# waiwera/waiwera

Measured on AMD Instinct MI355X. Metric: Newton steps/sec, 10M-cell eos_we (BCSR SpMV GB/s in roofline), higher is better.
Workload: dtype f64

## Files before the change

### waiwera_amd/csrc/context.hpp

```cpp
#pragma once
#include <hip/hip_runtime.h>
#include <string>
#include <type_traits>
#include <vector>
#include "../../include/waiwera_hip.h"
#include "devbuf.hpp"
#include "ilu_schedule.hpp"
#include "mesh_pattern.hpp"
#include "physics.hip.h"
#include "tile_schedule.hpp"

namespace wai {

__host__ __device__ __forceinline__ size_t ell_ld(size_t n) {
  size_t ld = (n + 511) & ~(size_t)511;
  if ((ld & 262143) == 0) ld += 512;
  return ld;
}
__host__ __device__ __forceinline__ size_t ell_rows(int bs, size_t n) {
  if (bs >= 3) return ell_ld(n);
  return n;
}
__host__ __device__ __forceinline__ size_t ell_ix1(int bs, size_t n, int r, int k, size_t i) {
  if (bs >= 3) return ((i >> 6) * (size_t)(bs * bs) + (size_t)(r * bs + k)) * 64 + (i & 63);
// ... 226 lines not shown
constexpr int MAX_TRACERS = 8;
constexpr int POST_OFF = 64;
constexpr unsigned long long POST_KEY = 0x5bd1e995a5a5c3c3ull;
struct Tracers {
  int nt = 0;
  int phase[MAX_TRACERS] = {0};
  double decay[MAX_TRACERS] = {0}, activation[MAX_TRACERS] = {0}, diffusion[MAX_TRACERS] = {0};
  double* bc = nullptr;
  double* inj = nullptr;
  double* rhsb = nullptr;
  int mode = 0;
  long long n_sweeps = 0;
  unsigned char kernarg_tail[136] = {0};
};
static_assert(sizeof(Tracers) == 408, "Tracers is a kernel argument (k_tracer_assemble_all, k_tracer_lhs): its size is part of their argument layout");
static_assert(std::is_trivially_copyable<Tracers>::value, "a kernel argument holds views, never an owner");

struct TracerForm {
  int method, it, nt, phase;
  double dt, ratio, decay, activation, diffusion;
};
static_assert(std::is_trivially_copyable<TracerForm>::value && std::is_trivially_copyable<ResForm>::value &&
              std::is_trivially_copyable<EosParams>::value, "a kernel argument holds views, never an owner");

constexpr int FIN_MAXF = 64;
struct Fin {
  int count = 0;
  int nb = 0;
  int nf = 1;
  double* part2 = nullptr;
  int slot0 = 0, nslots = 0;
  int phase = -1;
  int seq = 0;
  double* scal = nullptr;
  double* post = nullptr;
};
static_assert(std::is_trivially_copyable<Fin>::value, "a kernel argument holds views, never an owner");

struct Krylov {
  double* d_post = nullptr;
  int seq = 0;
  long long n_launch = 0, n_copy = 0;
  DevBuf<double> partials;
  DevBuf<double> partials2;
  DevBuf<unsigned> started;
  bool alpha_pending = false;
  int nb_max = 0;
  DevBuf<double> scal;
  PinnedBuf<double> h_scal;
  int nblocks = 0;
  int nb_pc = 0;
};

struct KrylovVecs {
  DevBuf<double> R, RP, P, V, S, T, tmp, X_own;
  double* X = nullptr;
  DevBuf<double> bl;
  DevBuf<double> basis;
  int basis_m = 0;
};

struct KspOpts {
  int type = WAI_KSP_BCGS, restart = 30, max_its = 10000;
  double rtol = 1.e-5, atol = 1.e-50;
};
struct PcOpts {
  int type = WAI_AUX_PC_FOLLOW, asm_overlap = 1, ilu_levels = 0, sub = WAI_SUB_ILU;
};

struct LinSys {
  Bcsr A;
  DevBuf<double> val, fdg;
  KspOpts ksp;
  PcOpts pc;
  int n = 0, nl = 0;
  KrylovVecs* kv = nullptr;
  AsmSystem as;
  bool net_blocks = false;
};

struct Gather {
  DevBuf<double> in;
  DevBuf<double> send;
  DevBuf<double> recv;
  DevBuf<double> out;
  DevBuf<double> counts;
  DevBuf<int> idx;
  DevBuf<int> claim;
  DevBuf<int> flag;
  size_t n_in = 0, n_send = 0, n_recv = 0, n_out = 0, n_counts = 0, n_idx = 0, n_claim = 0;
};

}

namespace wai {
struct LuBlocks {
  DevBuf<double> inv;
  DevBuf<size_t> inv_ptr;
  std::vector<size_t> h_inv_ptr;
  size_t total = 0;
  int bs = 0;
};
int launch_lu_apply(wai_ctx* c, int bs, const double* r, double* z);

struct Handles {
  hipStream_t stream = nullptr;
  Comm* comm = nullptr;
  hipEvent_t ev_scal = nullptr;
  hipStream_t comm_stream = nullptr;
  hipEvent_t ev_pack = nullptr, ev_halo = nullptr;
  hipEvent_t ev0 = nullptr, ev1 = nullptr, pev0 = nullptr, pev1 = nullptr;
  Handles() = default;
  Handles(const Handles&) = delete;
  ~Handles();
};
}

struct wai_ctx : wai::Handles {
  int device = 0;
  int n_cu = 256;
  size_t lds_per_block = 64 * 1024;
  int kind = 0, np = 0, df = 0, nmob = 0;
  bool salt = false;
  wai::EosParams ep{};
  wai_solver_opts opts{};
  int sub_pc = WAI_SUB_ILU;
  std::vector<int> pc_tiles;
  wai::DeviceMesh mesh;
  wai::Sources src;
  wai::Network net;
  std::vector<int> src_gidx;
  int src_nglobal = 0;
  wai::Pattern pat;
  wai::LinSys flow, aux, coupled;
  wai::KrylovVecs kv, kv_coupled;
  wai::IluSchedule ilu;
  wai::LuBlocks lu;
  wai::Krylov ks;
  wai::Tracers tr;
  wai::Gather gat;
  wai::DevBuf<double> tr_bc, tr_inj, tr_rhsb;
  wai::DevBuf<double> flu, flu_last_iter, flu_last_step, flu_pert;
  wai::DevBuf<double> hstep;
  wai::DevBuf<double> w_y, w_yold, w_delta, w_f, w_lhs, w_a, w_b, w_c;
  wai::DevBuf<int> d_flags;
  wai::PinnedBuf<int> h_flags;
  wai::DevBuf<double> d_red;
  wai::PinnedBuf<double> h_red;
  wai::DevBuf<double> stage[4];
  size_t stage_len = 0;
  struct EnvSw {
    bool fin_separate = false; bool no_col16 = false; bool scalar_kernels = false; bool iluk_level_path = false;
    bool asm_unfused = false; bool no_desc_share = false; bool no_pack = false;
  } env;
  int test_drop_wait = 0;
  int n_nbr = 0;
  std::vector<int> nbr_rank, send_ptr, recv_ptr;
  wai::DevBuf<int> d_send_idx; wai::DevBuf<double> d_sendbuf, d_recvbuf;
  int send_total = 0, max_dof_buf = 0;
  double fnorm0 = 0.0;
  int method = 0;
  double ratio = 0.0;
  wai::DevBuf<double> w_lhs2;
  int scheme = 0, taken = 0;
  double dt_last = 0.0;
  wai::DevBuf<double> w_hist;
  wai::DevBuf<double> w_hist_prev;
  double dt_last_prev = 0.0;
  bool can_reject = false;
  bool prof_on = false;
  bool last_iter_partial = false;
  double prof_ms[wai::KC_COUNT] = {0};
  long long prof_n[wai::KC_COUNT] = {0};
  std::string err;
  bool bc_set = false;
  int dbg = 0;
};

namespace wai {
int launch_eos(wai_ctx* c, const double* y, int first, int count, bool perturbed);
int launch_residual(wai_ctx* c, double dt, const double* lhs_old, double* f, double* lhs_out,
                    double* rhs_out, const int* only = nullptr, int n_only = 0);
int launch_jacobian(wai_ctx* c, double dt, const double* lhs_old);
int launch_transitions(wai_ctx* c, const double* y_old, double* search, double* y);
int launch_tracer_assemble(wai_ctx* c, const TracerForm& tf, const double* alx_last,
                           const double* alx_last2, double* b);
int launch_tracer_assemble_all(wai_ctx* c, int method, double dt, double ratio, const double* alx_last,
                               const double* alx_last2, double* b);
int launch_tracer_lhs(wai_ctx* c, double* Al);
int launch_separator(wai_ctx* c, double pressure, double* out);
int launch_face_fluxes(wai_ctx* c, const int* face_cells, double* out);
int launch_source_rates(wai_ctx* c, double* out, bool raw = false);
int launch_tracer_pick(wai_ctx* c, const double* X, int it, double* x);
int launch_tracer_put(wai_ctx* c, const double* x, int it, double* X);
int launch_tracer_alx(wai_ctx* c, const double* X, double* alx);
int launch_max_scaled(wai_ctx* c, const double* v, const double* scale, double tol, double* val,
                      int* idx);
int launch_fluid_aos(wai_ctx* c, const double* flu_soa, double* out_aos);
int launch_region_get(wai_ctx* c, double* out);
int launch_region_set(wai_ctx* c, const double* in, int first, int count);

int launch_spmv(wai_ctx* c, const Bcsr& M, const double* x, double* y);
int launch_ilu_factor_on(wai_ctx* c, const Bcsr& M, IluSchedule& s);
int launch_pc_on(wai_ctx* c, const Bcsr& M, const IluSchedule& s, bool spmv, const double* in, double* z,
                 int dot_mode, const double* aux, const int* list = nullptr, int nrun = 0, const Fin* fin = nullptr,
                 const double* in2 = nullptr, const Bcsr* F = nullptr, const int* row_map = nullptr);
int pc_kernel_kind(const wai_ctx* c, const Bcsr& M, const IluSchedule& s);
bool pc_axpy_capable(const wai_ctx* c, const Bcsr& M);
bool pc_axpy_default(const wai_ctx* c, const Bcsr& M);
int launch_big_solve(wai_ctx* c, const Bcsr& M, const IluSchedule& s, double* z);
int launch_sublu_solve(wai_ctx* c, const Bcsr& M, const IluSchedule& s, double* z);
bool sublu_vector_in_lds(const IluSchedule& s, int bs);
int launch_asm_gather_matrix(wai_ctx* c, const Bcsr& M, const AsmSystem& a);
int launch_pack_rows(wai_ctx* c, const Bcsr& M);
int launch_unpack_rows(wai_ctx* c, const Bcsr& M, const AsmSystem& a);
int launch_asm_gather(wai_ctx* c, const AsmSystem& a, const double* r);
int launch_asm_scatter(wai_ctx* c, const AsmSystem& a, double* z);
int vec_dots(wai_ctx* c, const double* a1, const double* b1, int slot1, const double* a2, const double* b2,
             int slot2, int n);
int launch_pc(wai_ctx* c, const Bcsr& M, bool spmv, const double* in, double* z, int dot_mode, const double* aux,
              const int* list = nullptr, int nrun = 0, const Fin* fin = nullptr, const double* in2 = nullptr);
Fin make_fin(wai_ctx* c, int slot0, int nslots, int phase, bool post = false);
inline Fin make_fin_dots(wai_ctx* c, int dot_mode, int phase, bool post = false) {
  return make_fin(c, pc_dot_slot0(dot_mode), pc_dot_nslots(dot_mode), phase, post);
}
int launch_ell_to_bcsr(wai_ctx* c, const Bcsr& M, double* bcsr);
int launch_dg_spmv(wai_ctx* c, const Bcsr& M, const double* x, double* y);
int launch_dg_factor(wai_ctx* c, const Bcsr& M, IluSchedule& s);
int launch_dg_pc(wai_ctx* c, const Bcsr& M, const IluSchedule& s, bool spmv, const double* in, double* z, const int* list, int nrun);
int launch_dg_big_solve(wai_ctx* c, const Bcsr& M, const IluSchedule& s, double* z);
int launch_dg_to_bcsr(wai_ctx* c, const Bcsr& M, double* bcsr);
int launch_bcsr_to_ell(wai_ctx* c, const double* bcsr, const Bcsr& M);
int vec_finalize(wai_ctx* c, int nb, int slot0, int nslots, int phase);
int vec_dot(wai_ctx* c, const double* a, const double* b, int n, int slot);
int partials_clear(wai_ctx* c, int slot0, int nslots);
int vec_copy(wai_ctx* c, double* dst, const double* src, size_t n);
int vec_zero(wai_ctx* c, double* dst, size_t n);
int vec_waxpy(wai_ctx* c, double* w, double alpha, const double* x, const double* y, int n);
int bcgs_scalars(wai_ctx* c, int phase, bool post = false);
int bcgs_update_xrp_derive(wai_ctx* c, const KrylovVecs& k, int n);
int bcgs_post(wai_ctx* c, int seq);
void read_env(wai_ctx* c);
int test_drop_partials(wai_ctx* c, int n);
int bcgs_update_p(wai_ctx* c, const KrylovVecs& k, int n);
int bcgs_update_s(wai_ctx* c, const KrylovVecs& k, int n);
int bcgs_update_xr(wai_ctx* c, const KrylovVecs& k, int n, bool dots = true, int fin_phase = -2, bool post = false);
int bcgs_update_xrp(wai_ctx* c, const KrylovVecs& k, int n);
int pack_halo_axpy(wai_ctx* c, const double* a, const double* b, int dof, hipStream_t stream = nullptr);
int gmres_mdot(wai_ctx* c, const double* basis, size_t ld, int n, const double* w, int k);
int gmres_maxpy_norm(wai_ctx* c, const double* basis, size_t ld, int n, double* w, int k);
int gmres_scale_to(wai_ctx* c, double* dst, const double* src, int slot_norm2, int n);
int gmres_update_x(wai_ctx* c, const double* basis, size_t ld, int n, double* x, const double* ycoef_host, int k);
int pack_halo(wai_ctx* c, const double* vec, int dof, hipStream_t stream = nullptr);
int unpack_halo(wai_ctx* c, double* vec, int dof, hipStream_t stream = nullptr);
}
```

### waiwera_amd/csrc/kernels_fused.hip

```cpp
#include "pc_generic.hip.h"
#include "pc_wide.hip.h"
#include "pc_park.hip.h"
#include "pc_rows.hip.h"
#include "pc_wave.hip.h"
#include "krylov_vec.hip.h"

namespace wai {

static inline int vgrid(int n) {
  int g = (n + TPB - 1) / TPB;
  return g > 1024 ? 1024 : (g < 1 ? 1 : g);
}

void read_env(wai_ctx* c) {
  c->env.fin_separate = getenv("WAI_FIN_SEPARATE") != nullptr;
  c->env.no_col16 = getenv("WAI_NO_COL16") != nullptr;
  c->env.scalar_kernels = getenv("WAI_BCGS_SCALAR_KERNELS") != nullptr;
  c->env.iluk_level_path = getenv("WAI_ILUK_LEVEL_PATH") != nullptr;
  c->env.asm_unfused = getenv("WAI_ASM_UNFUSED") != nullptr;
  c->env.no_desc_share = getenv("WAI_NO_DESC_SHARE") != nullptr;
  c->env.no_pack = getenv("WAI_NO_PACK") != nullptr;
}

int pc_kernel_kind(const wai_ctx* c, const Bcsr& J, const IluSchedule& s) {
  if (J.dg) return -1;
  if (s.wide) return 4;
  if (c->dbg) return 0;
  if (s.wave_kernel && J.bs >= 3) return 3;
  if (s.rows_kernel) return 2;
  if (park_serves(s, J.bs)) return 1;
  return 0;
}
static bool kind_composes(int kind) { return kind >= 1 && kind <= 3; }
bool pc_axpy_capable(const wai_ctx* c, const Bcsr& M) { return !c->ilu.big && kind_composes(pc_kernel_kind(c, M, c->ilu)); }
bool pc_axpy_default(const wai_ctx* c, const Bcsr& M) {
  if (c->ilu.big) return false;
  const int kind = pc_kernel_kind(c, M, c->ilu);
  return (kind == 1 && c->ilu.col16 && !c->env.no_col16) || kind == 3;
}

template <int BS>
static void launch_pc_bs(wai_ctx* c, const Bcsr& J, const IluSchedule& s, bool spmv, const double* in, double* z,
                         int dot_mode, const double* aux, const int* list, int nrun, const Fin* finp, const double* in2,
                         const Bcsr* F, const int* row_map) {
  const int which = !list ? 0 : (list == s.sub_int ? 1 : (list == s.sub_bnd ? 2 : -1));
  if (!list) { nrun = s.nsub; list = s.sub_order; }
  const bool with_fin = finp && dot_mode != 0;
  Fin fin;
  if (finp && dot_mode != 0) { fin = *finp; fin.count = nrun; fin.nb = s.nsub; fin.nf = fin_slices(s.nsub); }
  c->ks.n_launch++;
  const int grid = ((nrun + 7) / 8) * 8 + (with_fin ? fin.nf : 0), T = pc_threads(s);
  const size_t lds = ((size_t)T * BS + 80) * sizeof(double);
  auto sp_ax = [&](auto&& go) {
    if (spmv) with_flag(in2 != nullptr, [&](auto ax) { go(std::true_type{}, ax); });
    else go(std::false_type{}, std::false_type{});
  };
  const int kind = pc_kernel_kind(c, J, s);
  const double* scal = c->ks.scal;
  const int* rp = (size_t)J.nnzb * 10 < (size_t)J.n * J.W * 9 ? J.rowptr : nullptr;
  if (kind == 4) {
    constexpr int NSB = BS == 1 ? 8 : (BS == 2 ? 6 : 0);
    if constexpr (BS == 2) {
      if (F && row_map && s.max_nlu <= 3) {
        with_flag(spmv, [&](auto sp) {
          hipLaunchKernelGGL((k_pc_wide<2, decltype(sp)::value, true, 3, true>), grid, T, lds, c->stream, J.n, J.W, nrun, s.sub_ptr,
                             s.sub_nlev, s.row_infow, s.row_uoffw, J.col, rp, J.val, s.fval, in, z, aux, c->ks.partials, c->ks.nb_max,
                             dot_mode, 0, list, fin, F->col, F->n, row_map);
        });
        return;
      }
    }
    if constexpr (NSB > 0) {
      if (F && s.max_nlu <= NSB) {
        with_flag(spmv, [&](auto sp) {
          with_flag(row_map != nullptr, [&](auto map) {
            hipLaunchKernelGGL((k_pc_wide<BS, decltype(sp)::value, true, NSB, decltype(map)::value>), grid, T, lds, c->stream, J.n, J.W,
                               nrun, s.sub_ptr, s.sub_nlev, s.row_infow, s.row_uoffw, J.col, rp, J.val, s.fval, in, z, aux,
                               c->ks.partials, c->ks.nb_max, dot_mode, 0, list, fin, F->col, F->n, row_map);
          });
        });
        return;
      }
    }
    const size_t room = (size_t)64 * 1024 > lds ? (size_t)64 * 1024 - lds : 0;
    const int ucap = (int)std::min((size_t)s.max_ublocks_w, room / ((size_t)BS * BS * sizeof(double)));
    const size_t lds_w = lds + (size_t)ucap * BS * BS * sizeof(double);
    auto wide = [&](auto sp, auto fill, auto map) {
      hipLaunchKernelGGL((k_pc_wide<BS, decltype(sp)::value, decltype(fill)::value, 0, decltype(map)::value>), grid, T, lds_w, c->stream,
                         J.n, J.W, nrun, s.sub_ptr, s.sub_nlev, s.row_infow, s.row_uoffw, J.col, rp, J.val, s.fval, in, z, aux,
                         c->ks.partials, c->ks.nb_max, dot_mode, ucap, list, fin, F ? F->col : J.col, F ? F->n : J.n, row_map);
    };
    with_flag(spmv, [&](auto sp) {
      if (F && row_map) wide(sp, std::true_type{}, std::true_type{});
      else with_flag(F != nullptr, [&](auto fill) { wide(sp, fill, std::false_type{}); });
    });
    return;
  }
  if (kind == 3) {
    if constexpr (BS >= 3) {
      const int ngrp = (nrun + 3) / 4;
      const int pbase = (list && list == s.sub_bnd) ? (s.n_int + 3) / 4 : 0, nb_w = pbase + ngrp;
      if (with_fin) { fin.nb = nb_w; fin.nf = fin_slices(nb_w); }
      c->ks.nb_pc = nb_w;
      const int gridw = ((ngrp + 7) / 8) * 8 + (with_fin ? fin.nf : 0);
      const int per = 64 * BS + s.max_ublocks_w * BS * BS;
      const size_t lds_w = (size_t)4 * per * sizeof(double);
      Stagger stagger;
      stagger.ncu = c->n_cu;
      stagger.per_cu = std::max(1, (int)((size_t)160 * 1024 / (lds_w + 864)));
      stagger.ticks = 400;
      sp_ax([&](auto sp, auto ax) {
        hipLaunchKernelGGL((k_pc_wave<BS, decltype(sp)::value, decltype(ax)::value>), gridw, 256, lds_w, c->stream, J.n, J.W, nrun,
                           s.sub_ptr, s.sub_nlev, s.row_info, s.row_uoffw, J.col, s.fval, s.dinv, in, in2, scal, z, aux, c->ks.partials,
                           c->ks.nb_max, dot_mode, list, rp, s.sub_split, per, pbase, fin, stagger);
      });
      return;
    }
  }
  if (kind == 2) {
    const int TR = ((s.max_rows * BS + 63) / 64) * 64;
    const size_t lds_r = ((size_t)s.max_rows * BS + BS + 5 * 16 + 8) * sizeof(double);
    auto rows = [&](auto nlu) {
      sp_ax([&](auto sp, auto ax) {
        constexpr int NLU = decltype(nlu)::value;
        hipLaunchKernelGGL((k_pc_rows<BS, decltype(sp)::value, NLU, NLU, decltype(ax)::value>), grid, TR, lds_r, c->stream, J.n, J.W,
                           nrun, s.sub_ptr, s.sub_nlev, s.row_info, J.col, s.fval, s.dinv, in, in2, scal, z, aux, c->ks.partials,
                           c->ks.nb_max, dot_mode, list, rp, s.sub_split, fin);
      });
    };
    if (s.max_nlu <= 3) rows(std::integral_constant<int, 3>{});
    else rows(std::integral_constant<int, 4>{});
    return;
  }
  if constexpr (BS == 2) {
    if (kind == 1) {
      const size_t lds_park = lds + (size_t)s.max_ublocks * 4 * sizeof(double);
      Stagger stagger;
      stagger.ncu = c->n_cu;
      stagger.per_cu = std::max(1, std::min(3, (int)((size_t)160 * 1024 / (lds_park + 704))));
      stagger.ticks = 600;
      const bool on16 = s.col16 && !c->env.no_col16;
      const bool shared = on16 && s.sub_desc && !c->env.no_desc_share;
      const int* d_info = shared ? s.t_info.get() : s.row_info.get();
      const int* d_uoff = shared ? s.t_uoff.get() : s.row_uoff.get();
      const unsigned short* d_c16 = shared ? s.t_col16.get() : s.col16.get();
      const int* d_desc = shared ? s.sub_desc.get() : s.sub_ptr.get();
      if (shared && which >= 0 && s.pack_tab[which] && !c->env.no_pack) {
        const int ngrp = s.n_groups[which], gridp = ((ngrp + 7) / 8) * 8 + (with_fin ? fin.nf : 0);
        sp_ax([&](auto sp, auto ax) {
          hipLaunchKernelGGL((k_pc_park<decltype(sp)::value, decltype(ax)::value, true, true>), gridp, T, lds_park, c->stream,
                             J.n, J.W, ngrp, s.sub_ptr, s.sub_nlev, d_desc, d_info, d_uoff, J.col, d_c16, s.sub_seg, s.fval, s.dinv,
                             in, in2, scal, z, aux, c->ks.partials, c->ks.nb_max, dot_mode, s.pack_tab[which].get(), fin, stagger);
        });
        return;
      }
      with_flag(on16, [&](auto c16) {
        sp_ax([&](auto sp, auto ax) {
          hipLaunchKernelGGL((k_pc_park<decltype(sp)::value, decltype(ax)::value, decltype(c16)::value>), grid, T, lds_park, c->stream,
                             J.n, J.W, nrun, s.sub_ptr, s.sub_nlev, d_desc, d_info, d_uoff, J.col, d_c16, s.sub_seg, s.fval, s.dinv,
                             in, in2, scal, z, aux, c->ks.partials, c->ks.nb_max, dot_mode, list, fin, stagger);
        });
      });
      return;
    }
  }
  auto generic = [&](auto di) {
    with_flag(spmv, [&](auto sp) {
      with_flag(s.fast3, [&](auto fast) {
        hipLaunchKernelGGL((k_pc<BS, decltype(sp)::value, decltype(di)::value, decltype(fast)::value>), grid, T, lds, c->stream,
                           J.n, J.W, nrun, s.sub_ptr, s.sub_nlev, s.row_info, J.col, J.val, s.fval, s.dinv, in, z, aux,
                           c->ks.partials, c->ks.nb_max, dot_mode, c->dbg, list, fin);
      });
    });
  };
  if (s.diag_only && s.scaled) generic(std::integral_constant<int, 2>{});
  else if (s.diag_only) generic(std::integral_constant<int, 1>{});
  else generic(std::integral_constant<int, 0>{});
}

int launch_pc_on(wai_ctx* c, const Bcsr& M, const IluSchedule& s, bool spmv, const double* in, double* z,
                 int dot_mode, const double* aux, const int* list, int nrun, const Fin* fin, const double* in2, const Bcsr* F,
                 const int* row_map) {
  if (F && (!s.wide || M.dg || M.W > WMAX || (!row_map && F->n != M.n) || F->bs != M.bs)) { c->err = "a factor pattern of its own asked of a kernel that has none"; return -1; }
  if (row_map && !F) { c->err = "a row map without a factor pattern of its own"; return -1; }
  if (row_map && z == in) { c->err = "the fused PCASM application cannot run in place: a block reads rows another block writes"; return -1; }
  if (in2 && (!spmv || !kind_composes(pc_kernel_kind(c, M, s)))) { c->err = "composed input asked of a kernel that cannot form it"; return -1; }
  const Fin* fin_later = nullptr;
  if (fin && dot_mode != 0 && c->env.fin_separate) { fin_later = fin; fin = nullptr; }
  if (M.dg) {
    c->ks.n_launch++;
    if (launch_dg_pc(c, M, s, spmv, in, z, list, nrun)) return -1;
    if (dot_mode == PC_DOT_NONE) return 0;
    const int n = M.dg * M.n, s0 = pc_dot_slot0(dot_mode);
    if (dot_mode == PC_DOT_ZA || dot_mode == PC_DOT_ZZ) vec_dots(c, z, dot_mode == PC_DOT_ZA ? aux : z, s0, nullptr, nullptr, 0, n);
    else {
      vec_dots(c, in, z, s0, z, z, s0 + 1, n);
      if (dot_mode == PC_DOT_MERGED) { vec_dots(c, in, in, s0 + 2, in, aux, s0 + 3, n); vec_dots(c, z, aux, s0 + 4, nullptr, nullptr, 0, n); }
    }
    if (const Fin* f = fin ? fin : fin_later) {
      if (dot_mode == PC_DOT_MERGED) { vec_finalize(c, c->ks.nb_pc, s0, 4, -1); vec_finalize(c, c->ks.nb_pc, s0 + 4, 1, f->phase); }
      else vec_finalize(c, c->ks.nb_pc, s0, pc_dot_nslots(dot_mode), f->phase);
      if (f->seq > 0) bcgs_post(c, f->seq);
    }
    return 0;
  }
  c->ks.nb_pc = s.nsub;
  if (with_bs(M.bs, [&](auto bs) { launch_pc_bs<decltype(bs)::value>(c, M, s, spmv, in, z, dot_mode, aux, list, nrun, fin, in2, F, row_map); }) != 0)
    return -1;
  if (fin_later) {
    vec_finalize(c, c->ks.nb_pc, fin_later->slot0, fin_later->nslots, fin_later->phase);
    if (fin_later->seq > 0) bcgs_post(c, fin_later->seq);
  }
  return 0;
}
int launch_pc(wai_ctx* c, const Bcsr& M, bool spmv, const double* in, double* z, int dot_mode, const double* aux,
              const int* list, int nrun, const Fin* fin, const double* in2) {
  return launch_pc_on(c, M, c->ilu, spmv, in, z, dot_mode, aux, list, nrun, fin, in2);
}
Fin make_fin(wai_ctx* c, int slot0, int nslots, int phase, bool post) {
  Fin f;
  f.slot0 = slot0; f.nslots = nslots; f.phase = phase;
  f.scal = c->ks.scal; f.post = c->ks.d_post; f.part2 = c->ks.partials2;
  f.seq = post ? ++c->ks.seq : 0;
  return f;
}

int vec_finalize(wai_ctx* c, int nb, int slot0, int nslots, int phase) {
  const int T = nb > 256 ? 1024 : 256;
  c->ks.n_launch++;
  hipLaunchKernelGGL(k_finalize, 1, T, 0, c->stream, c->ks.partials, c->ks.nb_max, nb, slot0, nslots, c->ks.scal, phase);
  return 0;
}

int vec_dot(wai_ctx* c, const double* a, const double* b, int n, int slot) {
  const int g = vgrid(n);
  c->ks.n_launch++;
  hipLaunchKernelGGL(k_dot, g, TPB, 0, c->stream, a, b, n, c->ks.partials, c->ks.nb_max, slot);
  return vec_finalize(c, g, slot, 1, -1);
}
int vec_dots(wai_ctx* c, const double* a1, const double* b1, int slot1, const double* a2, const double* b2,
             int slot2, int n) {
  const int g = vgrid(n);
  c->ks.n_launch++;
  hipLaunchKernelGGL(k_dots, g, TPB, 0, c->stream, a1, b1, slot1, a2, b2, slot2, n, c->ks.partials, c->ks.nb_max);
  c->ks.nb_pc = g;
  return 0;
}
int partials_clear(wai_ctx* c, int slot0, int nslots) {
  const size_t tot = (size_t)nslots * std::max(c->ks.nb_max, (int)FIN_MAXF);
  c->ks.n_launch++;
  hipLaunchKernelGGL(k_partials_clear, (int)((tot + TPB - 1) / TPB), TPB, 0, c->stream, c->ks.partials, c->ks.partials2, c->ks.nb_max, slot0, nslots);
  return 0;
}
int vec_copy(wai_ctx* c, double* dst, const double* src, size_t n) {
  c->ks.n_copy++;
  return hipMemcpyAsync(dst, src, n * sizeof(double), hipMemcpyDeviceToDevice, c->stream) == hipSuccess ? 0 : -1;
}
int vec_zero(wai_ctx* c, double* dst, size_t n) {
  return hipMemsetAsync(dst, 0, n * sizeof(double), c->stream) == hipSuccess ? 0 : -1;
}
int vec_waxpy(wai_ctx* c, double* w, double alpha, const double* x, const double* y, int n) {
  c->ks.n_launch++;
  hipLaunchKernelGGL(k_waxpy, vgrid(n), TPB, 0, c->stream, w, alpha, x, y, n);
  return 0;
}
int bcgs_scalars(wai_ctx* c, int phase, bool post) {
  c->ks.n_launch++;
  hipLaunchKernelGGL(k_bcgs_scalars, 1, 64, 0, c->stream, c->ks.scal, phase, c->ks.d_post, post ? ++c->ks.seq : 0);
  return 0;
}
int test_drop_partials(wai_ctx* c, int n) {
  return hipMemcpyToSymbolAsync(HIP_SYMBOL(g_drop_partials), &n, sizeof(int), 0, hipMemcpyHostToDevice, c->stream) == hipSuccess &&
         hipStreamSynchronize(c->stream) == hipSuccess ? 0 : -1;
}
int bcgs_post(wai_ctx* c, int seq) {
  c->ks.n_launch++;
  hipLaunchKernelGGL(k_bcgs_scalars, 1, 64, 0, c->stream, c->ks.scal, -1, c->ks.d_post, seq);
  return 0;
}

int bcgs_update_p(wai_ctx* c, const KrylovVecs& k, int n) {
  c->ks.n_launch++;
  hipLaunchKernelGGL(k_bcgs_p, vgrid(n), TPB, 0, c->stream, k.P, k.R, k.V, n, c->ks.scal);
  return 0;
}
int bcgs_update_s(wai_ctx* c, const KrylovVecs& k, int n) {
  c->ks.n_launch++;
  hipLaunchKernelGGL(k_bcgs_s, vgrid(n), TPB, 0, c->stream, k.S, k.R, k.V, n, c->ks.scal);
  return 0;
}
int bcgs_update_xr(wai_ctx* c, const KrylovVecs& k, int n, bool dots, int fin_phase, bool post) {
  const int g = vgrid(n);
  Fin fin;
  if (dots && fin_phase >= -1) { fin = make_fin(c, S_DP2, 2, fin_phase, post); fin.count = g; fin.nb = g; fin.nf = fin_slices(g); }
  c->ks.n_launch++;
  if (dots && fin.count > 0 && c->env.fin_separate) {
    Fin none;
    hipLaunchKernelGGL(k_bcgs_xr<true>, g, TPB, 0, c->stream, k.X, k.R, k.P, k.S, k.T,
                       k.RP, n, c->ks.scal, c->ks.partials, c->ks.nb_max, none);
    c->ks.nblocks = g;
    vec_finalize(c, g, S_DP2, 2, fin_phase);
    if (fin.seq > 0) bcgs_post(c, fin.seq);
    return 0;
  }
  if (dots)
    hipLaunchKernelGGL(k_bcgs_xr<true>, g + (fin.count > 0 ? fin.nf : 0), TPB, 0, c->stream, k.X, k.R, k.P, k.S, k.T,
                       k.RP, n, c->ks.scal, c->ks.partials, c->ks.nb_max, fin);
  else
// ... 75 lines not shown
```

### waiwera_amd/csrc/pc_park.hip.h

```cpp
#pragma once
#include "reductions.hip.h"

namespace wai {

template <bool SPMV, bool AX, bool C16, bool PACK = false>
__global__ __launch_bounds__(512, 6) void k_pc_park(
    int n, int W, int nsub, const int* __restrict__ sub_ptr, const int* __restrict__ sub_nlev,
    const int* __restrict__ sub_desc, const int* __restrict__ row_info, const int* __restrict__ row_uoff, const int* __restrict__ col,
    const unsigned short* __restrict__ col16, const int* __restrict__ sub_seg,
    const double* __restrict__ sval, const double* __restrict__ dinv, const double* __restrict__ in,
    const double* __restrict__ in2, const double* __restrict__ scal,
    double* __restrict__ z, const double* __restrict__ aux, double* partials, int nb_max, int dot,
    const int* __restrict__ sub_list, Fin fin, Stagger stagger) {
  constexpr int BS = 2, BB = 4, MLU = 3;
  extern __shared__ __attribute__((aligned(16))) double lds[];
  if (fin_block(fin, partials, nb_max)) return;
  int s = xcd_remap(blockIdx.x, nsub);
  if (s >= nsub) return;
  int toff = 0, ubase = 0, nl_grp = 0;
  if constexpr (PACK) {
    const int w = __builtin_amdgcn_readfirstlane((int)threadIdx.x >> 6);
    const int4 rec = reinterpret_cast<const int4*>(sub_list)[(size_t)s * 8 + w];
    s = rec.x; toff = rec.y; ubase = rec.z; nl_grp = rec.w;
  } else {
    if (sub_list) s = sub_list[s];
  }
  const bool member = !PACK || s >= 0;
  const int lo = member ? sub_ptr[s] : 0, R = member ? sub_ptr[s + 1] - lo : 0;
  int dlo = lo;
  if constexpr (C16) dlo = member ? sub_desc[s] : 0;
  const int nl = PACK ? nl_grp : sub_nlev[s];
  const int nlf = nl & 0xffff, nlb = nl >> 16;
  const int tid = threadIdx.x, lob = lo - toff, i = lob + tid, di = dlo - toff + tid;
  const bool active = tid - toff < R;
  const double nalpha = AX ? -scal[S_ALPHA] : 0.0;
  stagger_start(stagger);
  double* ys = lds;
  double* upark = lds + (size_t)blockDim.x * BS + 80 + (size_t)ubase * BB;
  double Lf[MLU][BB];
  int Lc[MLU], Uc[MLU], lf = -1, lb = -1, uo = 0, nU = 0;
  double xin[BS] = {0.0, 0.0}, avp[BS] = {0.0, 0.0};
#pragma unroll
  for (int p = 0; p < MLU; p++) {
    Lc[p] = tid; Uc[p] = tid;
#pragma unroll
    for (int e = 0; e < BB; e++) Lf[p][e] = 0.0;
  }
  int lfirst = 0, dslot = 0, ulast = 0;
  int cgs[WMAX];
  if (active) {
    unpack_info(row_info[di], lfirst, dslot, ulast, lf, lb);
    uo = row_uoff[di];
    nU = ulast - dslot - 1;
    if constexpr (C16) {
      const int* sg = sub_seg + (size_t)s * 8;
      const int g0 = sg[0], g1 = sg[1], g2 = sg[2], g3 = sg[3], g4 = sg[4], g5 = sg[5], g6 = sg[6], g7 = sg[7];
      typedef unsigned wai_u4v __attribute__((ext_vector_type(4)));
      const wai_u4v pk = reinterpret_cast<const wai_u4v*>(col16)[di];
      const unsigned pw[4] = {pk.x, pk.y, pk.z, pk.w};
      unsigned cu[WMAX];
#pragma unroll
      for (int q = 0; q < WMAX; q++) cu[q] = (pw[q >> 1] >> (16 * (q & 1))) & 0xffffu;
#pragma unroll
      for (int q = 0; q < WMAX; q++) {
        const unsigned code = cu[q] >> 13;
        int b = g0;
        b = code == 1 ? g1 : b; b = code == 2 ? g2 : b; b = code == 3 ? g3 : b; b = code == 4 ? g4 : b;
        b = code == 5 ? g5 : b; b = code == 6 ? g6 : b; b = code == 7 ? g7 : b;
        cgs[q] = q < W ? b + (int)(cu[q] & 8191u) : i;
      }
    } else {
#pragma unroll
      for (int q = 0; q < WMAX; q++) {
        cgs[q] = i;
        if (q < W) cgs[q] = load_col(col, (size_t)q * n + i);
      }
    }
  }
  double acc[BS] = {0.0, 0.0};
  if (active) {
#pragma unroll
    for (int q = 0; q < WMAX; q++) {
      if (q < W) {
        const int cg = cgs[q];
        double blk[BB];
        load_block<BS>(sval, n, q, i, blk);
        if constexpr (SPMV) {
          double xv[BS];
          load_xs<BS, AX>(in, in2, nalpha, cg, xv);
          acc[0] += blk[0] * xv[0] + blk[1] * xv[1];
          acc[1] += blk[2] * xv[0] + blk[3] * xv[1];
          xin[0] = q == dslot ? xv[0] : xin[0];
          xin[1] = q == dslot ? xv[1] : xin[1];
        }
        const bool isl = (q >= lfirst) && (q < dslot), isu = (q > dslot) && (q < ulast);
#pragma unroll
        for (int p = 0; p < MLU; p++) {
          const bool tl = isl && (q - lfirst == p), tu = isu && (q - dslot - 1 == p);
          Lc[p] = tl ? cg - lob : Lc[p];
          Uc[p] = tu ? cg - lob : Uc[p];
#pragma unroll
          for (int e = 0; e < BB; e++) Lf[p][e] = tl ? blk[e] : Lf[p][e];
        }
        if (isu) {
          double* dst = upark + (size_t)(uo + (q - dslot - 1)) * BB;
          *reinterpret_cast<double2*>(dst) = make_double2(blk[0], blk[1]);
          *reinterpret_cast<double2*>(dst + 2) = make_double2(blk[2], blk[3]);
        }
      }
    }
    if constexpr (!SPMV) {
      double r[BS], dv[BB];
      load_x<BS>(in, i, r);
      load_pivot<BS>(dinv, n, i, dv);
      acc[0] = dv[0] * r[0] + dv[1] * r[1];
      acc[1] = dv[2] * r[0] + dv[3] * r[1];
      xin[0] = r[0]; xin[1] = r[1];
    }
    if (dot == PC_DOT_ZA || dot == PC_DOT_MERGED) load_x_stream<BS>(aux, i, avp);
  }
  if (active) *reinterpret_cast<double2*>(ys + tid * 2) = make_double2(acc[0], acc[1]);
  __syncthreads();
  auto gather3 = [&](const int (&cc)[MLU], const double (&ff)[MLU][BB], double* sum) {
    double2 yk[MLU];
#pragma unroll
    for (int p = 0; p < MLU; p++) yk[p] = *reinterpret_cast<const double2*>(ys + cc[p] * 2);
#pragma unroll
    for (int r = 0; r < BS; r++) {
      double part[MLU];
#pragma unroll
      for (int p = 0; p < MLU; p++) part[p] = ff[p][r * BS] * yk[p].x + ff[p][r * BS + 1] * yk[p].y;
      sum[r] = (part[0] + part[1]) + part[2];
    }
  };
  for (int lev = 1; lev < nlf; lev++) {
    if (lf == lev) {
      const double2 a = *reinterpret_cast<const double2*>(ys + tid * 2);
      double sum[BS];
      gather3(Lc, Lf, sum);
      *reinterpret_cast<double2*>(ys + tid * 2) = make_double2(a.x - sum[0], a.y - sum[1]);
    }
    __syncthreads();
  }
#pragma unroll
  for (int p = 0; p < MLU; p++) {
    const bool have = p < nU;
    const double* src = upark + (size_t)(uo + (have ? p : 0)) * BB;
    const double2 u0 = *reinterpret_cast<const double2*>(src), u1 = *reinterpret_cast<const double2*>(src + 2);
    Lf[p][0] = have ? u0.x : 0.0; Lf[p][1] = have ? u0.y : 0.0;
    Lf[p][2] = have ? u1.x : 0.0; Lf[p][3] = have ? u1.y : 0.0;
  }
  double out[BS] = {0.0, 0.0};
  for (int lev = 0; lev < nlb; lev++) {
    if (lb == lev) {
      const double2 a = *reinterpret_cast<const double2*>(ys + tid * 2);
      double sum[BS];
      gather3(Uc, Lf, sum);
      out[0] = a.x - sum[0];
      out[1] = a.y - sum[1];
      *reinterpret_cast<double2*>(ys + tid * 2) = make_double2(out[0], out[1]);
    }
    if (lev + 1 < nlb) __syncthreads();
  }
  if (active) store_z2(z, (size_t)i, out[0], out[1]);
  if (dot != 0) {
    double* red = lds + (size_t)blockDim.x * BS;
    double v[5] = {0.0, 0.0, 0.0, 0.0, 0.0};
    pc_row_dots<BS, true, false>(dot, v, out, active, [&](double (&x)[BS]) { x[0] = xin[0]; x[1] = xin[1]; },
                                 [&](double (&a)[BS]) { a[0] = avp[0]; a[1] = avp[1]; });
    __syncthreads();
    if constexpr (PACK) pc_reduce_dots_waves(dot, v, red, partials, nb_max, s, toff >> 6, (R + 63) >> 6);
    else pc_reduce_dots(dot, v, red, partials, nb_max, s);
  }
}

}
```

### waiwera_amd/csrc/reductions.hip.h

```cpp
#pragma once
#include "linalg_device.hip.h"

namespace wai {

typedef unsigned wai_u4 __attribute__((ext_vector_type(4)));
__device__ __forceinline__ void post_scalars(const double* scal, double* post, int seq) {
  const double v0 = scal[S_DP2], v1 = 8.0 * (double)seq + scal[S_BREAK];
  const unsigned long long chk = (unsigned long long)__double_as_longlong(v0) ^ (unsigned long long)__double_as_longlong(v1) ^ POST_KEY;
#if defined(__gfx942__) || defined(__gfx950__)
  wai_u4 w;
  w.x = (unsigned)__double2loint(v0); w.y = (unsigned)__double2hiint(v0);
  w.z = (unsigned)__double2loint(v1); w.w = (unsigned)__double2hiint(v1);
  asm volatile("global_store_dwordx4 %0, %1, off sc0 sc1" : : "v"(post), "v"(w) : "memory");
#else
  __hip_atomic_store(reinterpret_cast<unsigned long long*>(post), (unsigned long long)__double_as_longlong(v0), __ATOMIC_RELAXED, __HIP_MEMORY_SCOPE_SYSTEM);
  __hip_atomic_store(reinterpret_cast<unsigned long long*>(post) + 1, (unsigned long long)__double_as_longlong(v1), __ATOMIC_RELAXED, __HIP_MEMORY_SCOPE_SYSTEM);
#endif
  __hip_atomic_store(reinterpret_cast<unsigned long long*>(post) + 2, chk, __ATOMIC_RELAXED, __HIP_MEMORY_SCOPE_SYSTEM);
}
__device__ __forceinline__ void derive_merged(double* s) {
  const double st = s[S_D1], tt = s[S_D2], ss = s[S_DP2], srp = s[S_RHONEW], trp = s[S_W2];
  if (tt == 0.0) { s[S_BREAK] = 2.0; s[S_OMEGA] = 0.0; }
  else s[S_OMEGA] = st / tt;
  const double om = s[S_OMEGA];
// ... 39 lines not shown
  const int per = (nb + nf - 1) / nf;
  lo = f * per; hi = lo + per < nb ? lo + per : nb;
  if (lo > nb) lo = nb;
}
__device__ __forceinline__ void sum_slice(unsigned long long* p0, int nb_max, int lo, int hi, int ns, bool wait,
                                          double* scal, double* res) {
  __shared__ __attribute__((aligned(16))) double fsm[FIN_MAXS][16];
  constexpr int CH = 2;
  const int len = hi - lo, VT = len > 256 ? 1024 : 256;
  __syncthreads();
  bool gave_up = false;
  for (int v = threadIdx.x; v < VT; v += blockDim.x) {
    double t[FIN_MAXS];
#pragma unroll
    for (int s = 0; s < FIN_MAXS; s++) t[s] = 0.0;
    for (int i0 = lo + v; i0 < hi; i0 += VT * CH) {
      unsigned long long u[FIN_MAXS][CH];
#pragma unroll
      for (int s = 0; s < FIN_MAXS; s++)
#pragma unroll
        for (int k = 0; k < CH; k++) {
          const int i = i0 + k * VT;
          u[s][k] = (s < ns && i < hi) ? __hip_atomic_load(p0 + (size_t)s * nb_max + i, __ATOMIC_RELAXED, __HIP_MEMORY_SCOPE_AGENT) : 0ull;
        }
      for (int spin = 0; wait && !gave_up && spin < (1 << 22); spin++) {
        bool any = false;
#pragma unroll
        for (int s = 0; s < FIN_MAXS; s++)
#pragma unroll
          for (int k = 0; k < CH; k++) any |= (s < ns && i0 + k * VT < hi && u[s][k] == FIN_EMPTY);
        if (!any) break;
        __builtin_amdgcn_s_sleep(8);
#pragma unroll
        for (int s = 0; s < FIN_MAXS; s++)
#pragma unroll
          for (int k = 0; k < CH; k++) {
            const int i = i0 + k * VT;
            if (s < ns && i < hi && u[s][k] == FIN_EMPTY)
              u[s][k] = __hip_atomic_load(p0 + (size_t)s * nb_max + i, __ATOMIC_RELAXED, __HIP_MEMORY_SCOPE_AGENT);
          }
      }
#pragma unroll
      for (int s = 0; s < FIN_MAXS; s++)
#pragma unroll
        for (int k = 0; k < CH; k++) {
          const int i = i0 + k * VT;
          if (s < ns && i < hi) {
            if (u[s][k] == FIN_EMPTY) {
              gave_up = true;
              __hip_atomic_store(&scal[S_BREAK], 4.0, __ATOMIC_RELAXED, __HIP_MEMORY_SCOPE_AGENT);
              __builtin_amdgcn_fence(__ATOMIC_RELEASE, "agent");
            }
            __hip_atomic_store(p0 + (size_t)s * nb_max + i, FIN_EMPTY, __ATOMIC_RELAXED, __HIP_MEMORY_SCOPE_AGENT);
            t[s] += __longlong_as_double((long long)u[s][k]);
          }
        }
    }
#pragma unroll
    for (int s = 0; s < FIN_MAXS; s++) {
      const double ts = wave_sum(t[s]);
      if ((v & 63) == 0) fsm[s][v >> 6] = ts;
    }
  }
  __syncthreads();
  if ((int)threadIdx.x < ns) {
    double tot = 0.0;
    for (int w = 0; w < (VT >> 6); w++) tot += fsm[threadIdx.x][w];
    res[threadIdx.x] = tot;
  }
  __syncthreads();
}
__device__ __forceinline__ void sum_partials(const double* partials, int nb_max, int nb, int slot0, int nslots,
                                             double* scal, bool wait) {
  __shared__ __attribute__((aligned(16))) double res[8], tot[8];
  const int nf = fin_slices(nb);
  for (int sb = 0; sb < nslots; sb += FIN_MAXS) {
    const int ns = min(nslots - sb, FIN_MAXS);
    unsigned long long* p0 = reinterpret_cast<unsigned long long*>(const_cast<double*>(partials)) + (size_t)(slot0 + sb) * nb_max;
    if ((int)threadIdx.x < ns) tot[threadIdx.x] = 0.0;
    for (int f = 0; f < nf; f++) {
      int lo, hi;
      fin_slice_range(nb, nf, f, lo, hi);
      sum_slice(p0, nb_max, lo, hi, ns, wait, scal, res);
      if ((int)threadIdx.x < ns) tot[threadIdx.x] = nf == 1 ? res[threadIdx.x] : tot[threadIdx.x] + res[threadIdx.x];
    }
    if ((int)threadIdx.x < ns) scal[slot0 + sb + threadIdx.x] = tot[threadIdx.x];
    __syncthreads();
  }
}
__device__ int g_drop_partials = 0;
__device__ __forceinline__ void store_partial(double* p, double t) {
  if (blockIdx.x == 0 && __hip_atomic_load(&g_drop_partials, __ATOMIC_RELAXED, __HIP_MEMORY_SCOPE_AGENT) > 0 &&
      atomicSub(&g_drop_partials, 1) > 0)
    return;
  __hip_atomic_store(p, t, __ATOMIC_RELAXED, __HIP_MEMORY_SCOPE_AGENT);
}
__device__ __forceinline__ bool fin_block(const Fin& f, const double* partials, int nb_max) {
  if (f.count == 0 || (int)blockIdx.x < (int)gridDim.x - f.nf) return false;
  __shared__ __attribute__((aligned(16))) double res[8];
  const int me = (int)blockIdx.x - ((int)gridDim.x - f.nf);
  const bool last = me == f.nf - 1;
  unsigned long long* p0 = reinterpret_cast<unsigned long long*>(const_cast<double*>(partials)) + (size_t)f.slot0 * nb_max;
  unsigned long long* q0 = reinterpret_cast<unsigned long long*>(f.part2) + (size_t)f.slot0 * FIN_MAXF;
  int lo, hi;
  fin_slice_range(f.nb, f.nf, me, lo, hi);
  sum_slice(p0, nb_max, lo, hi, f.nslots, true, f.scal, res);
  if (f.nf == 1) {
    if ((int)threadIdx.x < f.nslots) f.scal[f.slot0 + threadIdx.x] = res[threadIdx.x];
  } else {
    if ((int)threadIdx.x < f.nslots) store_partial(f.part2 + (size_t)(f.slot0 + threadIdx.x) * FIN_MAXF + me, res[threadIdx.x]);
    if (!last) return true;
    if (threadIdx.x < 64) {
      const int t = (int)threadIdx.x;
      unsigned long long u[FIN_MAXS];
#pragma unroll
      for (int s2 = 0; s2 < FIN_MAXS; s2++)
        u[s2] = (s2 < f.nslots && t < f.nf) ? __hip_atomic_load(q0 + (size_t)s2 * FIN_MAXF + t, __ATOMIC_RELAXED, __HIP_MEMORY_SCOPE_AGENT) : 0ull;
      for (int spin = 0; spin < (1 << 22); spin++) {
        bool any = false;
#pragma unroll
        for (int s2 = 0; s2 < FIN_MAXS; s2++) any |= (s2 < f.nslots && t < f.nf && u[s2] == FIN_EMPTY);
        if (!any) break;
        __builtin_amdgcn_s_sleep(8);
#pragma unroll
        for (int s2 = 0; s2 < FIN_MAXS; s2++)
          if (s2 < f.nslots && t < f.nf && u[s2] == FIN_EMPTY)
            u[s2] = __hip_atomic_load(q0 + (size_t)s2 * FIN_MAXF + t, __ATOMIC_RELAXED, __HIP_MEMORY_SCOPE_AGENT);
      }
#pragma unroll
      for (int s2 = 0; s2 < FIN_MAXS; s2++) {
        if (s2 < f.nslots) {
          if (t < f.nf) {
            if (u[s2] == FIN_EMPTY) __hip_atomic_store(&f.scal[S_BREAK], 4.0, __ATOMIC_RELAXED, __HIP_MEMORY_SCOPE_AGENT);
            __hip_atomic_store(q0 + (size_t)s2 * FIN_MAXF + t, FIN_EMPTY, __ATOMIC_RELAXED, __HIP_MEMORY_SCOPE_AGENT);
          }
          const double v = __longlong_as_double((long long)u[s2]);
          double tot = 0.0;
          for (int g = 0; g < f.nf; g++) tot += __shfl(v, g);
          if (t == 0) f.scal[f.slot0 + s2] = tot;
        }
      }
    }
  }
  __syncthreads();
  if (threadIdx.x == 0) {
    __threadfence_block();
    if (__hip_atomic_load(&f.scal[S_BREAK], __ATOMIC_RELAXED, __HIP_MEMORY_SCOPE_AGENT) == 4.0) f.scal[S_BREAK] = 4.0;
    if (f.phase >= 0) derive_scalars(f.scal, f.phase);
    if (f.seq > 0) post_scalars(f.scal, f.post, f.seq);
  }
  return true;
}

struct Stagger { int ticks = 0, ncu = 256, per_cu = 3; };
static_assert(std::is_trivially_copyable<Stagger>::value, "a kernel argument holds views, never an owner");
__device__ __forceinline__ void stagger_start(const Stagger& st) {
  if (st.ticks > 0 && (int)blockIdx.x < st.ncu * st.per_cu) {
    const unsigned long long t0 = wall_clock64(), wait = (unsigned long long)((int)blockIdx.x / st.ncu) * (unsigned long long)st.ticks;
    while (wall_clock64() - t0 < wait) __builtin_amdgcn_s_sleep(32);
  }
}

template <int NS>
__device__ __forceinline__ void wg_reduce_store(double (&v)[NS], double* red, double* partials,
                                                int nb_max, int slot0, int blk) {
  const int lane = threadIdx.x & 63, w = threadIdx.x >> 6, nw = (blockDim.x + 63) >> 6;
#pragma unroll
  for (int s = 0; s < NS; s++) {
    const double t = wave_sum(v[s]);
    if (lane == 0) red[s * 16 + w] = t;
  }
  __syncthreads();
  if (nw >= NS) {
    if (lane == 0 && w < NS) {
      double t = 0.0;
      for (int q = 0; q < nw; q++) t += red[w * 16 + q];
      store_partial(partials + (size_t)(slot0 + w) * nb_max + blk, t);
    }
    return;
  }
  if (threadIdx.x == 0) {
#pragma unroll
    for (int s = 0; s < NS; s++) {
      double t = 0.0;
      for (int q = 0; q < nw; q++) t += red[s * 16 + q];
      store_partial(partials + (size_t)(slot0 + s) * nb_max + blk, t);
    }
  }
}
__device__ __forceinline__ void pc_reduce_dots(int mode, double (&v)[5], double* red, double* partials, int nb_max, int blk) {
  const int slot0 = pc_dot_slot0(mode);
  if (mode == PC_DOT_MERGED) wg_reduce_store<5>(v, red, partials, nb_max, slot0, blk);
  else if (mode == PC_DOT_XZ) { double v2[2] = {v[0], v[1]}; wg_reduce_store<2>(v2, red, partials, nb_max, slot0, blk); }
  else { double v1[1] = {v[0]}; wg_reduce_store<1>(v1, red, partials, nb_max, slot0, blk); }
}

template <int NS>
__device__ __forceinline__ void wg_reduce_store_waves(double (&v)[NS], double* red, double* partials, int nb_max, int slot0,
                                                      int blk, int w0, int nwm) {
  const int lane = threadIdx.x & 63, w = threadIdx.x >> 6;
#pragma unroll
  for (int s = 0; s < NS; s++) {
    const double t = wave_sum(v[s]);
    if (lane == 0) red[s * 16 + w] = t;
  }
  __syncthreads();
  if (blk < 0 || lane != 0) return;
  const int k = w - w0;
  if (nwm >= NS) {
    if (k < NS) {
      double t = 0.0;
      for (int q = w0; q < w0 + nwm; q++) t += red[k * 16 + q];
      store_partial(partials + (size_t)(slot0 + k) * nb_max + blk, t);
    }
    return;
  }
  if (k == 0) {
#pragma unroll
    for (int s = 0; s < NS; s++) {
      double t = 0.0;
      for (int q = w0; q < w0 + nwm; q++) t += red[s * 16 + q];
      store_partial(partials + (size_t)(slot0 + s) * nb_max + blk, t);
    }
  }
}
__device__ __forceinline__ void pc_reduce_dots_waves(int mode, double (&v)[5], double* red, double* partials, int nb_max, int blk,
                                                     int w0, int nwm) {
  const int slot0 = pc_dot_slot0(mode);
  if (mode == PC_DOT_MERGED) wg_reduce_store_waves<5>(v, red, partials, nb_max, slot0, blk, w0, nwm);
  else if (mode == PC_DOT_XZ) { double v2[2] = {v[0], v[1]}; wg_reduce_store_waves<2>(v2, red, partials, nb_max, slot0, blk, w0, nwm); }
  else { double v1[1] = {v[0]}; wg_reduce_store_waves<1>(v1, red, partials, nb_max, slot0, blk, w0, nwm); }
}

template <int N, bool SUM, bool GUARD2, class GetX, class GetA>
__device__ __forceinline__ void pc_row_dots(int mode, double (&v)[5], const double (&o)[N], bool active, GetX get_x,
                                            GetA get_a) {
  auto dot = [&](int q, const double (&p)[N], const double (&r)[N]) {
    if constexpr (SUM) {
      double t = p[0] * r[0];
#pragma unroll
      for (int k = 1; k < N; k++) t += p[k] * r[k];
      v[q] = t;
    } else {
#pragma unroll
      for (int k = 0; k < N; k++) v[q] += p[k] * r[k];
    }
  };
  double x[N], a[N];
  if (mode == PC_DOT_ZA) {
    if (active) { get_a(a); dot(0, o, a); }
  } else if (mode == PC_DOT_XZ) {
    if (active || !GUARD2) { get_x(x); dot(0, x, o); dot(1, o, o); }
  } else if (mode == PC_DOT_MERGED) {
    if (active) { get_x(x); get_a(a); dot(0, x, o); dot(1, o, o); dot(2, x, x); dot(3, x, a); dot(4, o, a); }
  } else {
    dot(0, o, o);
  }
}

template <int NS>
__device__ __forceinline__ void block_reduce_store(double (&v)[NS], double* partials, int nb_max,
                                                   const int* slots) {
  __shared__ double sm[NS][TPB / 64];
#pragma unroll
  for (int s = 0; s < NS; s++) {
    const double t = wave_sum(v[s]);
    if ((threadIdx.x & 63) == 0) sm[s][threadIdx.x >> 6] = t;
  }
  __syncthreads();
  if (threadIdx.x == 0) {
#pragma unroll
    for (int s = 0; s < NS; s++) {
      double t = 0.0;
#pragma unroll
      for (int w = 0; w < TPB / 64; w++) t += sm[s][w];
      store_partial(partials + (size_t)slots[s] * nb_max + blockIdx.x, t);
    }
  }
}

}
```

Before: 5.446.

## Stage SpMV input vector in LDS for in-block columns of park preconditioner kernel

Adds a STAGE variant of the parked ILU preconditioner kernel. Each row's SpMV input (with the fused axpy applied) goes into LDS, and in-subdomain neighbour columns are read from LDS instead of global memory. The first far-column operand and the first value block are prefetched early to overlap their latency, and the dot products are computed with explicit FMA ordering. It is enabled by default for composed (in2) calls on the shared-descriptor path, adding LDS barriers and register pressure.

```diff
diff --git a/waiwera_amd/csrc/context.hpp b/waiwera_amd/csrc/context.hpp
--- a/waiwera_amd/csrc/context.hpp
+++ b/waiwera_amd/csrc/context.hpp
@@ -402,6 +402,7 @@
   struct EnvSw {
     bool fin_separate = false; bool no_col16 = false; bool scalar_kernels = false; bool iluk_level_path = false;
     bool asm_unfused = false; bool no_desc_share = false; bool no_pack = false;
+    int park_stage = -1;
   } env;
   int test_drop_wait = 0;
   int n_nbr = 0;
diff --git a/waiwera_amd/csrc/kernels_fused.hip b/waiwera_amd/csrc/kernels_fused.hip
--- a/waiwera_amd/csrc/kernels_fused.hip
+++ b/waiwera_amd/csrc/kernels_fused.hip
@@ -20,6 +20,19 @@
   c->env.asm_unfused = getenv("WAI_ASM_UNFUSED") != nullptr;
   c->env.no_desc_share = getenv("WAI_NO_DESC_SHARE") != nullptr;
   c->env.no_pack = getenv("WAI_NO_PACK") != nullptr;
+  const char* st = getenv("WAI_PARK_STAGE");
+  c->env.park_stage = st && (st[0] == '0' || st[0] == '1') ? st[0] - '0' : -1;
+}
+
+#ifndef WAI_PARK_STAGE_COMPOSED
+#define WAI_PARK_STAGE_COMPOSED 1
+#endif
+#ifndef WAI_PARK_STAGE_FIRST
+#define WAI_PARK_STAGE_FIRST 0
+#endif
+static bool park_staged(const wai_ctx* c, bool composed) {
+  if (c->env.park_stage >= 0) return c->env.park_stage == 1;
+  return composed ? WAI_PARK_STAGE_COMPOSED != 0 : WAI_PARK_STAGE_FIRST != 0;
 }
 
 int pc_kernel_kind(const wai_ctx* c, const Bcsr& J, const IluSchedule& s) {
@@ -145,8 +158,17 @@
       const int* d_uoff = shared ? s.t_uoff.get() : s.row_uoff.get();
       const unsigned short* d_c16 = shared ? s.t_col16.get() : s.col16.get();
       const int* d_desc = shared ? s.sub_desc.get() : s.sub_ptr.get();
+      const bool stage = shared && spmv && park_staged(c, in2 != nullptr);
+      auto staged = [&](auto pack, int g, int count, const int* lst) {
+        with_flag(in2 != nullptr, [&](auto ax) {
+          hipLaunchKernelGGL((k_pc_park<true, decltype(ax)::value, true, decltype(pack)::value, true>), g, T, lds_park, c->stream,
+                             J.n, J.W, count, s.sub_ptr, s.sub_nlev, d_desc, d_info, d_uoff, J.col, d_c16, s.sub_seg, s.fval, s.dinv,
+                             in, in2, scal, z, aux, c->ks.partials, c->ks.nb_max, dot_mode, lst, fin, stagger);
+        });
+      };
       if (shared && which >= 0 && s.pack_tab[which] && !c->env.no_pack) {
         const int ngrp = s.n_groups[which], gridp = ((ngrp + 7) / 8) * 8 + (with_fin ? fin.nf : 0);
+        if (stage) { staged(std::true_type{}, gridp, ngrp, s.pack_tab[which].get()); return; }
         sp_ax([&](auto sp, auto ax) {
           hipLaunchKernelGGL((k_pc_park<decltype(sp)::value, decltype(ax)::value, true, true>), gridp, T, lds_park, c->stream,
                              J.n, J.W, ngrp, s.sub_ptr, s.sub_nlev, d_desc, d_info, d_uoff, J.col, d_c16, s.sub_seg, s.fval, s.dinv,
@@ -154,6 +176,7 @@
         });
         return;
       }
+      if (stage) { staged(std::false_type{}, grid, nrun, list); return; }
       with_flag(on16, [&](auto c16) {
         sp_ax([&](auto sp, auto ax) {
           hipLaunchKernelGGL((k_pc_park<decltype(sp)::value, decltype(ax)::value, decltype(c16)::value>), grid, T, lds_park, c->stream,
diff --git a/waiwera_amd/csrc/pc_park.hip.h b/waiwera_amd/csrc/pc_park.hip.h
--- a/waiwera_amd/csrc/pc_park.hip.h
+++ b/waiwera_amd/csrc/pc_park.hip.h
@@ -3,7 +3,7 @@
 
 namespace wai {
 
-template <bool SPMV, bool AX, bool C16, bool PACK = false>
+template <bool SPMV, bool AX, bool C16, bool PACK = false, bool STAGE = false>
 __global__ __launch_bounds__(512, 6) void k_pc_park(
     int n, int W, int nsub, const int* __restrict__ sub_ptr, const int* __restrict__ sub_nlev,
     const int* __restrict__ sub_desc, const int* __restrict__ row_info, const int* __restrict__ row_uoff, const int* __restrict__ col,
@@ -13,6 +13,7 @@
     double* __restrict__ z, const double* __restrict__ aux, double* partials, int nb_max, int dot,
     const int* __restrict__ sub_list, Fin fin, Stagger stagger) {
   constexpr int BS = 2, BB = 4, MLU = 3;
+  static_assert(!STAGE || (SPMV && C16), "the staged operand is the operator's, on the 16-bit column indices");
   extern __shared__ __attribute__((aligned(16))) double lds[];
   if (fin_block(fin, partials, nb_max)) return;
   int s = xcd_remap(blockIdx.x, nsub);
@@ -48,10 +49,16 @@
   }
   int lfirst = 0, dslot = 0, ulast = 0;
   int cgs[WMAX];
+  [[maybe_unused]] double own2[BS], blk0[BB], xr0[BS], xv0[BS];
+  [[maybe_unused]] bool far0 = false;
   if (active) {
     unpack_info(row_info[di], lfirst, dslot, ulast, lf, lb);
     uo = row_uoff[di];
     nU = ulast - dslot - 1;
+    if constexpr (STAGE) {
+      load_x<BS>(in, i, xin);
+      if constexpr (AX) load_x<BS>(in2, i, own2);
+    }
     if constexpr (C16) {
       const int* sg = sub_seg + (size_t)s * 8;
       const int g0 = sg[0], g1 = sg[1], g2 = sg[2], g3 = sg[3], g4 = sg[4], g5 = sg[5], g6 = sg[6], g7 = sg[7];
@@ -76,6 +83,23 @@
         if (q < W) cgs[q] = load_col(col, (size_t)q * n + i);
       }
     }
+    if constexpr (STAGE) {
+      load_block<BS>(sval, n, 0, i, blk0);
+      if constexpr (AX) {
+#pragma unroll
+        for (int k = 0; k < BS; k++) xin[k] = __builtin_fma(nalpha, own2[k], xin[k]);
+      }
+      *reinterpret_cast<double2*>(ys + tid * 2) = make_double2(xin[0], xin[1]);
+      far0 = lfirst > 0;
+      if (far0) {
+        load_x<BS>(in, cgs[0], xr0);
+        if constexpr (AX) load_x<BS>(in2, cgs[0], xv0);
+      }
+    }
+  }
+  if constexpr (STAGE) {
+    lds_barrier();
+    __builtin_amdgcn_s_waitcnt(0x0f70);
   }
   double acc[BS] = {0.0, 0.0};
   if (active) {
@@ -84,8 +108,25 @@
       if (q < W) {
         const int cg = cgs[q];
         double blk[BB];
-        load_block<BS>(sval, n, q, i, blk);
-        if constexpr (SPMV) {
+        if constexpr (STAGE) {
+          if (q == 0) {
+#pragma unroll
+            for (int e = 0; e < BB; e++) blk[e] = blk0[e];
+          } else load_block<BS>(sval, n, q, i, blk);
+          const bool inb = (q >= lfirst) && (q < ulast);
+          const double2 sv = *reinterpret_cast<const double2*>(ys + ((inb && q != dslot) ? cg - lob : tid) * 2);
+          double xv[BS] = {q == dslot ? xin[0] : sv.x, q == dslot ? xin[1] : sv.y};
+          if (!inb) {
+            if (q == 0) {
+              asm volatile("" : "+v"(xr0[0]), "+v"(xr0[1]));
+              xv[0] = xr0[0]; xv[1] = xr0[1];
+              if constexpr (AX) { xv[0] = __builtin_fma(nalpha, xv0[0], xv[0]); xv[1] = __builtin_fma(nalpha, xv0[1], xv[1]); }
+            } else load_xs<BS, AX>(in, in2, nalpha, cg, xv);
+          }
+          acc[0] += blk[0] * xv[0] + blk[1] * xv[1];
+          acc[1] += blk[2] * xv[0] + blk[3] * xv[1];
+        } else load_block<BS>(sval, n, q, i, blk);
+        if constexpr (SPMV && !STAGE) {
           double xv[BS];
           load_xs<BS, AX>(in, in2, nalpha, cg, xv);
           acc[0] += blk[0] * xv[0] + blk[1] * xv[1];
@@ -119,6 +160,7 @@
     }
     if (dot == PC_DOT_ZA || dot == PC_DOT_MERGED) load_x_stream<BS>(aux, i, avp);
   }
+  if constexpr (STAGE) lds_barrier();
   if (active) *reinterpret_cast<double2*>(ys + tid * 2) = make_double2(acc[0], acc[1]);
   __syncthreads();
   auto gather3 = [&](const int (&cc)[MLU], const double (&ff)[MLU][BB], double* sum) {
@@ -166,6 +208,19 @@
   if (dot != 0) {
     double* red = lds + (size_t)blockDim.x * BS;
     double v[5] = {0.0, 0.0, 0.0, 0.0, 0.0};
+    if constexpr (STAGE) {
+      auto hi = [](const double (&p)[BS], const double (&r)[BS]) { return __builtin_fma(p[0], r[0], p[1] * r[1]); };
+      auto lo = [](const double (&p)[BS], const double (&r)[BS]) { return __builtin_fma(p[1], r[1], p[0] * r[0]); };
+      if (dot == PC_DOT_ZA) {
+        if (active) v[0] = hi(out, avp);
+      } else if (dot == PC_DOT_XZ) {
+        v[0] = hi(xin, out); v[1] = hi(out, out);
+      } else if (dot == PC_DOT_MERGED) {
+        if (active) { v[0] = hi(xin, out); v[1] = hi(out, out); v[2] = lo(xin, xin); v[3] = lo(xin, avp); v[4] = hi(out, avp); }
+      } else {
+        v[0] = hi(out, out);
+      }
+    } else
     pc_row_dots<BS, true, false>(dot, v, out, active, [&](double (&x)[BS]) { x[0] = xin[0]; x[1] = xin[1]; },
                                  [&](double (&a)[BS]) { a[0] = avp[0]; a[1] = avp[1]; });
     __syncthreads();
diff --git a/waiwera_amd/csrc/reductions.hip.h b/waiwera_amd/csrc/reductions.hip.h
--- a/waiwera_amd/csrc/reductions.hip.h
+++ b/waiwera_amd/csrc/reductions.hip.h
@@ -215,6 +215,12 @@
   return true;
 }
 
+__device__ __forceinline__ void lds_barrier() {
+  __builtin_amdgcn_fence(__ATOMIC_RELEASE, "workgroup", "local");
+  __builtin_amdgcn_s_barrier();
+  __builtin_amdgcn_fence(__ATOMIC_ACQUIRE, "workgroup", "local");
+}
+
 struct Stagger { int ticks = 0, ncu = 256, per_cu = 3; };
 static_assert(std::is_trivially_copyable<Stagger>::value, "a kernel argument holds views, never an owner");
 __device__ __forceinline__ void stagger_start(const Stagger& st) {
```

After: 5.533 (median of 6 runs). 1.6% higher.
